# PacificBiosciences/minorseq

Hardware: AMD Instinct MI355X
Metric: aligned CCS reads/sec through juliet call+phase (higher is better)
Workload: dtype u3 symbols as bit planes / u32 counts / f64 p-values; 1 GPU; configs[2]: 100000 CCS reads x 3000 bp reference per GPU, pileup + Fisher-exact + phasing (96% major + four 1% minor haplotypes, sub 1.75e-4, del 1.3e-3, N 2e-2); every resident batch holds different reads; reads_per_gpu=100000, ref_columns_per_gpu=3000, parallelism=single GPU, batches_per_launch=8, launches_in_flight=4, resident_batches=32, variants_called=5, haplotypes=5, windows_verified_in_loop=270

## Files before the change

### minorseq_amd/csrc/kernels_pileup.hip

```cpp
#include <stdlib.h>
#include <string.h>

#include "call_eval.h"
#include "deviation_index.h"
#include "jl_internal.h"

namespace {


__device__ __forceinline__ uint32_t wave_sum(uint32_t v)
{
    v += (uint32_t)__builtin_amdgcn_update_dpp(0, (int)v, 0xB1, 0xF, 0xF, true);
    v += (uint32_t)__builtin_amdgcn_update_dpp(0, (int)v, 0x4E, 0xF, 0xF, true);
    v += (uint32_t)__builtin_amdgcn_update_dpp(0, (int)v, 0x141, 0xF, 0xF, true);
    v += (uint32_t)__builtin_amdgcn_update_dpp(0, (int)v, 0x140, 0xF, 0xF, true);
    v += (uint32_t)__builtin_amdgcn_update_dpp(0, (int)v, 0x142, 0xA, 0xF, false);
    v += (uint32_t)__builtin_amdgcn_update_dpp(0, (int)v, 0x143, 0xC, 0xF, false);
    return v;
}

typedef uint32_t u32x4 __attribute__((ext_vector_type(4)));

#define JL_CHUNK_META(ncols, startf, halo) ((uint32_t)(ncols) | ((uint32_t)(startf) << 4) | ((uint32_t)(halo) << 16))

typedef uint32_t u32x2 __attribute__((ext_vector_type(2)));
constexpr uint32_t plane_tile_bytes(int nq) { return 256u * 4u * (uint32_t)nq; }
constexpr uint32_t plane_flush_tiles(int nq) { return 1023u / (32u * (uint32_t)nq); }

template <int W, int NQ>
struct ptile_regs {
    uint32_t d[W + 2][3][NQ];
};

template <int W, int NQ, bool FAST>
__device__ __forceinline__ void load_ptile(ptile_regs<W, NQ> &r, const uint8_t JL_AS1 *planes, uint64_t plane_stride, uint32_t n_cols,
                                           uint32_t c0, uint32_t ncols, uint64_t off, bool need_halo)
{
#pragma unroll
    for (int j = 0; j < W + 2; ++j) {
        if (FAST && j >= 3) continue;
        const bool live = FAST ? true : (c0 + j < n_cols) && ((uint32_t)j < ncols || (need_halo && (uint32_t)j < ncols + 2u));
        if (live) {
            const uint8_t JL_AS1 *base = planes + (uint64_t)(c0 + j) * 3u * plane_stride + off;
#pragma unroll
            for (int k = 0; k < 3; ++k) {
                if (NQ == 2) {
                    const u32x2 v = __builtin_nontemporal_load((const u32x2 JL_AS1 *)(base + (uint64_t)k * plane_stride));
                    r.d[j][k][0] = v.x;
                    r.d[j][k][1] = v.y;
                } else {
                    const u32x4 v = __builtin_nontemporal_load((const u32x4 JL_AS1 *)(base + (uint64_t)k * plane_stride));
                    r.d[j][k][0] = v.x;
                    r.d[j][k][1] = v.y;
                    r.d[j][k][NQ - 2] = v.z;
                    r.d[j][k][NQ - 1] = v.w;
                }
            }
        } else {
#pragma unroll
            for (int q = 0; q < NQ; ++q) {
                r.d[j][0][q] = 0u;
                r.d[j][1][q] = r.d[j][2][q] = 0xFFFFFFFFu;
            }
        }
    }
}

template <int W, int NQ, bool FAST>
__device__ __forceinline__ void pileup_planes_stream(const uint8_t JL_AS1 *planes, uint64_t plane_stride, uint32_t n_cols,
                                                     uint32_t n_tiles, uint32_t c0, uint32_t ncols, uint32_t startf, bool need_halo,
                                                     const uint32_t (&g)[W + 2], uint32_t (*s_hist)[64], uint32_t (*s_col)[6],
                                                     uint32_t *s_match)
{
    constexpr uint32_t TILE = plane_tile_bytes(NQ);
    const uint32_t tid = threadIdx.x;
    const bool last_lane = (tid & 63u) == 63u;
    const uint64_t lane_off = (uint64_t)tid * 4u * NQ;
    uint32_t sh[W + 2], sl[W + 2];
#pragma unroll
    for (int j = 0; j < W + 2; ++j) {
        sh[j] = (g[j] & 2u) ? 0xFFFFFFFFu : 0u;
        sl[j] = (g[j] & 1u) ? 0xFFFFFFFFu : 0u;
    }

    uint32_t tile = blockIdx.y;
    ptile_regs<W, NQ> nxt;
    bool nxt_live = false;
    if (tile < n_tiles) {
        const uint64_t off = (uint64_t)tile * TILE + lane_off;
        nxt_live = off < plane_stride;
        if (nxt_live) load_ptile<W, NQ, FAST>(nxt, planes, plane_stride, n_cols, c0, ncols, off, need_halo);
    }

    while (tile < n_tiles) {
        uint32_t acc[W][6];
        uint32_t match[W];
#pragma unroll
        for (int j = 0; j < W; ++j) {
            match[j] = 0;
#pragma unroll
            for (int k = 0; k < 6; ++k) acc[j][k] = 0;
        }
        uint32_t reads = 0;

        for (uint32_t it = 0; it < plane_flush_tiles(NQ) && tile < n_tiles; ++it, tile += gridDim.y) {
            const ptile_regs<W, NQ> cur = nxt;
            const bool live = nxt_live;
            const uint32_t tn = tile + gridDim.y;
            nxt_live = false;
            if (tn < n_tiles) {
                const uint64_t off = (uint64_t)tn * TILE + lane_off;
                nxt_live = off < plane_stride;
                if (nxt_live) load_ptile<W, NQ, FAST>(nxt, planes, plane_stride, n_cols, c0, ncols, off, need_halo);
            }
            if (!live) continue;
            reads += 32u * NQ;
#pragma unroll
            for (int j = 0; j < W; ++j) {
                if (FAST ? j < 3 : (uint32_t)j < ncols) {
#pragma unroll
                    for (int q = 0; q < NQ; ++q) {
                        const uint32_t b0 = cur.d[j][0][q], b1 = cur.d[j][1][q], b2 = cur.d[j][2][q];
                        acc[j][0] += __popc(b0);
                        acc[j][1] += __popc(b1);
                        acc[j][2] += __popc(b2);
                        acc[j][3] += __popc(b0 & b1);
                        acc[j][4] += __popc(b0 & b2);
                        acc[j][5] += __popc(b1 & b2);
                    }
                }
            }
#pragma unroll
            for (int j = 0; j < W; ++j) {
                if (FAST ? j == 0 : (startf & (1u << j)) != 0) {
#pragma unroll
                    for (int q = 0; q < NQ; ++q) {
                        const uint32_t inv = cur.d[j][2][q] | cur.d[j + 1][2][q] | cur.d[j + 2][2][q];
                        const uint32_t x = (cur.d[j][1][q] ^ sh[j]) | (cur.d[j][0][q] ^ sl[j]) | (cur.d[j + 1][1][q] ^ sh[j + 1]) |
                                           (cur.d[j + 1][0][q] ^ sl[j + 1]) | (cur.d[j + 2][1][q] ^ sh[j + 2]) | (cur.d[j + 2][0][q] ^ sl[j + 2]);
                        match[j] += __popc(~(x | inv));
                        uint32_t rest = x & ~inv;
                        while (rest) {
                            const int b = __ffs((int)rest) - 1;
                            rest &= rest - 1;
                            const uint32_t idx = (((cur.d[j][1][q] >> b) & 1u) << 5) | (((cur.d[j][0][q] >> b) & 1u) << 4) |
                                                 (((cur.d[j + 1][1][q] >> b) & 1u) << 3) | (((cur.d[j + 1][0][q] >> b) & 1u) << 2) |
                                                 (((cur.d[j + 2][1][q] >> b) & 1u) << 1) | ((cur.d[j + 2][0][q] >> b) & 1u);
                            atomicAdd(&s_hist[j][idx], 1u);
                        }
                    }
                }
            }
        }

#pragma unroll
        for (int j = 0; j < W; ++j) {
            if (FAST && j >= 3) continue;
            const uint32_t nT = acc[j][3], nN = acc[j][4], nU = acc[j][5];
            const uint32_t nC = acc[j][0] - nT - nN, nG = acc[j][1] - nT - nU, nD = acc[j][2] - nN - nU;
            const uint32_t nA = reads - (nC + nG + nT + nD + nN + nU);
            const uint32_t p0 = wave_sum(nA | (nC << 16));
            const uint32_t p1 = wave_sum(nG | (nT << 16));
            const uint32_t p2 = wave_sum(nD | (nN << 16));
            const bool starts = FAST ? j == 0 : (startf & (1u << j)) != 0;
            uint32_t p3 = 0;
            if (starts) p3 = wave_sum(match[j]);
            if (last_lane && (uint32_t)j < ncols) {
                if (p0 & 0xFFFFu) atomicAdd(&s_col[j][0], p0 & 0xFFFFu);
                if (p0 >> 16) atomicAdd(&s_col[j][1], p0 >> 16);
                if (p1 & 0xFFFFu) atomicAdd(&s_col[j][2], p1 & 0xFFFFu);
                if (p1 >> 16) atomicAdd(&s_col[j][3], p1 >> 16);
                if (p2 & 0xFFFFu) atomicAdd(&s_col[j][4], p2 & 0xFFFFu);
                if (p2 >> 16) atomicAdd(&s_col[j][5], p2 >> 16);
                if (starts && p3) atomicAdd(&s_match[j], p3);
            }
        }
    }
}

template <int W, bool FOLD>
__device__ __forceinline__ void pileup_tail(uint32_t (*s_hist)[64], uint32_t (*s_col)[6], uint32_t *s_match, const uint32_t (&g)[W + 2],
                                            uint32_t c0, uint32_t ncols, uint32_t startf, uint32_t JL_AS1 *counts, uint32_t JL_AS1 *hist,
                                            const jl_win_fold *fold)
{
    const uint32_t tid = threadIdx.x;
    const bool excl = gridDim.y == 1;
    if (tid < W * 6) {
        const uint32_t j = tid / 6u, k = tid - j * 6u;
        const uint32_t v = s_col[j][k];
        if (j < ncols) {
            if (excl) counts[(uint64_t)(c0 + j) * 6u + k] = v;
            else if (v) atomicAdd((uint32_t *)(counts + (uint64_t)(c0 + j) * 6u + k), v);
        }
    }
    if (tid < W && (startf & (1u << tid))) {
        const uint32_t j = tid;
        const uint32_t seed = (g[j] << 4) | (g[j + 1] << 2) | g[j + 2];
        s_hist[j][seed] += s_match[j];
    }
    __syncthreads();
    for (uint32_t i = tid; i < W * 64; i += 256) {
        const uint32_t j = i >> 6;
        const uint32_t v = s_hist[j][i & 63u];
        if (startf & (1u << j)) {
            if (excl) hist[(uint64_t)(c0 + j) * 64u + (i & 63u)] = v;
            else if (v) atomicAdd((uint32_t *)(hist + (uint64_t)(c0 + j) * 64u + (i & 63u)), v);
        }
    }
    if (FOLD) {
        const jl_win_call &c = fold->c;
        if (blockIdx.x == 0 && tid == 0 && c.meta) {
            c.meta->n_occupied = 0;
            c.meta->overflow = 0;
            jl_phase_summary z = {0, 0, 0, 0, 0, 0, 0, 0};
            c.meta->summary = z;
        }
        const uint32_t wid = tid >> 6, lane = tid & 63u;
#pragma unroll
        for (int j = 0; j < W; ++j) {
            if (((uint32_t)j & 3u) != wid || !(startf & (1u << j))) continue;
            const uint32_t col = c0 + (uint32_t)j;
            const uint32_t h = s_hist[j][lane];
            for (uint32_t p = fold->col_head[col]; p != 0xFFFFFFFFu; p = fold->pos_next[p])
                jl_call_position<false>(c.A, p, col, h, c.pos_refcfg[p], c.pos_gene[p], c.pos_codon[p], c.drm, c.called, c.staged);
        }
    }
}

template <int W, int NQ, bool FOLD>
__device__ __forceinline__ void pileup_planes_body(const uint8_t JL_AS1 *planes, uint64_t plane_stride, uint32_t n_cols, uint32_t n_tiles,
                                                   const uint2 JL_AS1 *chunks, const uint32_t JL_AS1 *guess32, uint32_t JL_AS1 *counts,
                                                   uint32_t JL_AS1 *hist, const jl_win_fold *fold)
{
    __shared__ uint32_t s_hist[W][64];
    __shared__ uint32_t s_col[W][6];
    __shared__ uint32_t s_match[W];
    const uint32_t tid = threadIdx.x;
    const uint2 rec = chunks[blockIdx.x];
    const uint32_t c0 = rec.x;
    const uint32_t ncols = rec.y & 15u;
    const uint32_t startf = (rec.y >> 4) & 0xFFFu;
    const bool need_halo = ((rec.y >> 16) & 1u) != 0;
    constexpr int NG = (W + 2 + 3 + 3) / 4;
    uint32_t gw[NG];
#pragma unroll
    for (int k = 0; k < NG; ++k) gw[k] = guess32[(c0 >> 2) + k];
    uint32_t g[W + 2];
#pragma unroll
    for (int j = 0; j < W + 2; ++j) {
        const uint32_t b = (c0 & 3u) + (uint32_t)j;
        uint32_t word = gw[0];
#pragma unroll
        for (int k = 1; k < NG; ++k)
            if ((b >> 2) == (uint32_t)k) word = gw[k];
        g[j] = (word >> (8u * (b & 3u))) & 3u;
    }
    for (uint32_t i = tid; i < W * 64; i += 256) (&s_hist[0][0])[i] = 0;
    if (tid < W * 6) (&s_col[0][0])[tid] = 0;
    if (tid < W) s_match[tid] = 0;
    __syncthreads();
    if (W == 3 && rec.y == JL_CHUNK_META(3, 1, 0))
        pileup_planes_stream<W, NQ, true>(planes, plane_stride, n_cols, n_tiles, c0, ncols, startf, need_halo, g, s_hist, s_col, s_match);
    else
        pileup_planes_stream<W, NQ, false>(planes, plane_stride, n_cols, n_tiles, c0, ncols, startf, need_halo, g, s_hist, s_col, s_match);
    __syncthreads();
    pileup_tail<W, FOLD>(s_hist, s_col, s_match, g, c0, ncols, startf, counts, hist, fold);
}

template <int W, int NQ>
__global__ __launch_bounds__(256) void pileup_planes_kernel(const uint8_t *__restrict__ planes, uint64_t plane_stride, uint32_t n_cols,
                                                            uint32_t n_tiles, const uint2 *__restrict__ chunks,
                                                            const uint32_t *__restrict__ guess32, uint32_t *__restrict__ counts,
                                                            uint32_t *__restrict__ hist)
{
    pileup_planes_body<W, NQ, false>((const uint8_t JL_AS1 *)planes, plane_stride, n_cols, n_tiles, (const uint2 JL_AS1 *)chunks,
                                     (const uint32_t JL_AS1 *)guess32, (uint32_t JL_AS1 *)counts, (uint32_t JL_AS1 *)hist, nullptr);
}

template <int W, int NQ>
__global__ __launch_bounds__(256) void pileup_planes_group_kernel(jl_pileup_group_args args)
{
    const jl_win_pileup &w = args.w[blockIdx.z];
    if (blockIdx.x >= w.n_chunks) return;
    pileup_planes_body<W, NQ, false>((const uint8_t JL_AS1 *)w.msa, w.plane_stride, w.n_cols, w.n_tiles, (const uint2 JL_AS1 *)w.chunks,
                                     (const uint32_t JL_AS1 *)w.guess32, (uint32_t JL_AS1 *)w.counts, (uint32_t JL_AS1 *)w.hist, nullptr);
}

template <int W, int NQ>
__global__ __launch_bounds__(256) void pileup_fold_kernel(jl_win_pileup w, jl_win_fold f)
{
    pileup_planes_body<W, NQ, true>((const uint8_t JL_AS1 *)w.msa, w.plane_stride, w.n_cols, w.n_tiles, (const uint2 JL_AS1 *)w.chunks,
                                    (const uint32_t JL_AS1 *)w.guess32, (uint32_t JL_AS1 *)w.counts, (uint32_t JL_AS1 *)w.hist, &f);
}

template <int W, int NQ>
__global__ __launch_bounds__(256) void pileup_fold_group_kernel(jl_pileup_fold_group_args args)
{
    const jl_win_pileup &w = args.w[blockIdx.z];
    if (blockIdx.x >= w.n_chunks) return;
    pileup_planes_body<W, NQ, true>((const uint8_t JL_AS1 *)w.msa, w.plane_stride, w.n_cols, w.n_tiles, (const uint2 JL_AS1 *)w.chunks,
                                    (const uint32_t JL_AS1 *)w.guess32, (uint32_t JL_AS1 *)w.counts, (uint32_t JL_AS1 *)w.hist, &args.f[blockIdx.z]);
}

#ifndef JL_IX_FOLD_DEPTH
#define JL_IX_FOLD_DEPTH 8
#endif
template <int DEPTH>
__device__ __forceinline__ void index_stream(const uint32_t JL_AS1 *list, uint32_t E, uint32_t (*s_hist)[64], uint32_t (*s_col)[6])
{
    static_assert(DEPTH >= 1 && DEPTH <= 8, "rounds held in registers");
    constexpr uint32_t FLUSH_BATCHES = JL_IX_FLUSH_ROUNDS / (uint32_t)DEPTH;
    static_assert(FLUSH_BATCHES >= 1u && FLUSH_BATCHES * (uint32_t)DEPTH <= JL_IX_FLUSH_ROUNDS, "a 9-bit field never above 511");
    const uint32_t tid = threadIdx.x;
    const bool last_lane = (tid & 63u) == 63u;
    const u32x4 JL_AS1 *src = (const u32x4 JL_AS1 *)list;
    const uint32_t n_rounds = (E + 4u * 256u - 1u) / (4u * 256u);
    u32x4 buf[DEPTH];
#pragma unroll
    for (int k = 0; k < DEPTH; ++k) {
        buf[k] = u32x4{0u, 0u, 0u, 0u};
        if (((uint32_t)k * 256u + tid) * 4u < E) buf[k] = __builtin_nontemporal_load(src + (size_t)k * 256u + tid);
    }
    uint32_t r = 0;
    while (r < n_rounds) {
        unsigned long long acc[3] = {0ull, 0ull, 0ull};
        for (uint32_t it = 0; it < FLUSH_BATCHES && r < n_rounds; ++it, r += (uint32_t)DEPTH) {
#pragma unroll
            for (int k = 0; k < DEPTH; ++k) {
                if (r + (uint32_t)k >= n_rounds) break;
                const u32x4 cur = buf[k];
                const uint32_t first = ((r + (uint32_t)k) * 256u + tid) * 4u;
                const uint32_t nfirst = first + (uint32_t)DEPTH * 4u * 256u;
                if (nfirst < E) buf[k] = __builtin_nontemporal_load(src + (size_t)(r + (uint32_t)k + (uint32_t)DEPTH) * 256u + tid);
                const uint32_t e4[4] = {cur.x, cur.y, cur.z, cur.w};
#pragma unroll
                for (int i = 0; i < 4; ++i) {
                    if (first + (uint32_t)i >= E) continue;
                    const uint32_t e = e4[i];
                    const uint32_t a = (e >> 6) & 7u, b = (e >> 3) & 7u, c = e & 7u;
                    acc[0] += 1ull << (JL_IX_FIELD_BITS * a);
                    acc[1] += 1ull << (JL_IX_FIELD_BITS * b);
                    acc[2] += 1ull << (JL_IX_FIELD_BITS * c);
                    if ((e & 0x124u) == 0u) atomicAdd(&s_hist[0][(a << 4) | (b << 2) | c], 1u);
                }
            }
        }
#pragma unroll
        for (int j = 0; j < 3; ++j) {
            const uint32_t m = (1u << JL_IX_FIELD_BITS) - 1u;
            uint32_t p[3];
#pragma unroll
            for (int k = 0; k < 3; ++k)
                p[k] = wave_sum(((uint32_t)(acc[j] >> (JL_IX_FIELD_BITS * 2u * k)) & m) | (((uint32_t)(acc[j] >> (JL_IX_FIELD_BITS * (2u * k + 1u))) & m) << 16));
            if (last_lane) {
#pragma unroll
                for (int k = 0; k < 3; ++k) {
                    if (p[k] & 0xFFFFu) atomicAdd(&s_col[j][2 * k], p[k] & 0xFFFFu);
                    if (p[k] >> 16) atomicAdd(&s_col[j][2 * k + 1], p[k] >> 16);
                }
            }
        }
    }
}

__device__ __forceinline__ void index_dense_stream(const uint8_t JL_AS1 *planes, uint64_t plane_stride, uint32_t c0, const uint32_t (&g)[5],
                                                   uint32_t (*s_hist)[64], uint32_t (*s_col)[6], uint32_t *s_match)
{
    const uint32_t tid = threadIdx.x;
    const bool last_lane = (tid & 63u) == 63u;
    const uint32_t n_words = (uint32_t)(plane_stride / 4u);
    const uint32_t JL_AS1 *base = (const uint32_t JL_AS1 *)(planes + (uint64_t)c0 * 3u * plane_stride);
    const uint64_t row = plane_stride / 4u;
    uint32_t acc[3][6], match = 0, reads = 0;
#pragma unroll
    for (int j = 0; j < 3; ++j)
#pragma unroll
        for (int k = 0; k < 6; ++k) acc[j][k] = 0;
    for (uint32_t w = tid; w < n_words; w += 256u) {
        uint32_t d[3][3];
#pragma unroll
        for (int j = 0; j < 3; ++j)
#pragma unroll
            for (int k = 0; k < 3; ++k) d[j][k] = base[(uint64_t)(3 * j + k) * row + w];
        reads += 32u;
        uint32_t inv = 0, x = 0;
#pragma unroll
        for (int j = 0; j < 3; ++j) {
            const uint32_t b0 = d[j][0], b1 = d[j][1], b2 = d[j][2];
            acc[j][0] += __popc(b0);
            acc[j][1] += __popc(b1);
            acc[j][2] += __popc(b2);
            acc[j][3] += __popc(b0 & b1);
            acc[j][4] += __popc(b0 & b2);
            acc[j][5] += __popc(b1 & b2);
            inv |= b2;
            x |= (b1 ^ ((g[j] & 2u) ? 0xFFFFFFFFu : 0u)) | (b0 ^ ((g[j] & 1u) ? 0xFFFFFFFFu : 0u));
        }
        match += __popc(~(x | inv));
        uint32_t rest = x & ~inv;
        while (rest) {
            const int b = __ffs((int)rest) - 1;
            rest &= rest - 1;
            const uint32_t idx = (((d[0][1] >> b) & 1u) << 5) | (((d[0][0] >> b) & 1u) << 4) | (((d[1][1] >> b) & 1u) << 3) |
                                 (((d[1][0] >> b) & 1u) << 2) | (((d[2][1] >> b) & 1u) << 1) | ((d[2][0] >> b) & 1u);
            atomicAdd(&s_hist[0][idx], 1u);
        }
    }
#pragma unroll
    for (int j = 0; j < 3; ++j) {
        const uint32_t nT = acc[j][3], nN = acc[j][4], nU = acc[j][5];
        const uint32_t nC = acc[j][0] - nT - nN, nG = acc[j][1] - nT - nU, nD = acc[j][2] - nN - nU;
        const uint32_t nA = reads - (nC + nG + nT + nD + nN + nU);
        const uint32_t v[6] = {wave_sum(nA), wave_sum(nC), wave_sum(nG), wave_sum(nT), wave_sum(nD), wave_sum(nN)};
        if (last_lane) {
#pragma unroll
            for (int k = 0; k < 6; ++k)
                if (v[k]) atomicAdd(&s_col[j][k], v[k]);
        }
    }
    const uint32_t ms = wave_sum(match);
    if (last_lane && ms) atomicAdd(&s_match[0], ms);
}

template <bool FOLD>
__device__ __forceinline__ void pileup_index_body(const uint8_t JL_AS1 *planes, uint64_t plane_stride, uint32_t n_reads, const uint4 JL_AS1 *tab,
                                                  const uint32_t JL_AS1 *entries, const uint8_t JL_AS1 *seed, uint32_t JL_AS1 *counts,
                                                  uint32_t JL_AS1 *hist, const jl_win_fold *fold)
{
    __shared__ uint32_t s_hist[3][64];
    __shared__ uint32_t s_col[3][6];
    __shared__ uint32_t s_match[3];
    const uint32_t tid = threadIdx.x;
    const uint4 rec = tab[blockIdx.x];
    const uint32_t c0 = rec.x;
    const uint32_t g[5] = {seed[c0] & 3u, seed[c0 + 1u] & 3u, seed[c0 + 2u] & 3u, 0u, 0u};
    for (uint32_t i = tid; i < 3 * 64; i += 256) (&s_hist[0][0])[i] = 0;
    if (tid < 3 * 6) (&s_col[0][0])[tid] = 0;
    if (tid < 3) s_match[tid] = 0;
    __syncthreads();
    if (rec.z != 0xFFFFFFFFu) {
        index_stream<FOLD ? JL_IX_FOLD_DEPTH : 1>(entries + rec.y, rec.z, s_hist, s_col);
        if (tid < 3) atomicAdd(&s_col[tid][g[tid]], n_reads - rec.z);
        if (tid == 3) s_match[0] = n_reads - rec.z;
    } else {
        index_dense_stream(planes, plane_stride, c0, g, s_hist, s_col, s_match);
    }
    __syncthreads();
    pileup_tail<3, FOLD>(s_hist, s_col, s_match, g, c0, 3u, 1u, counts, hist, fold);
}

#define JL_INDEX_BODY(FOLD, w, f)                                                                                                     \
    pileup_index_body<FOLD>((const uint8_t JL_AS1 *)(w).msa, (w).plane_stride, (w).n_reads, (const uint4 JL_AS1 *)(w).tab,            \
                            (const uint32_t JL_AS1 *)(w).entries, (const uint8_t JL_AS1 *)(w).seed, (uint32_t JL_AS1 *)(w).counts,     \
                            (uint32_t JL_AS1 *)(w).hist, f)

__global__ __launch_bounds__(256) void pileup_index_kernel(jl_win_index w) { JL_INDEX_BODY(false, w, nullptr); }
__global__ __launch_bounds__(256) void pileup_index_fold_kernel(jl_win_index w, jl_win_fold f) { JL_INDEX_BODY(true, w, &f); }
__global__ __launch_bounds__(256) void pileup_index_group_kernel(jl_index_group_args args)
{
    const jl_win_index &w = args.w[blockIdx.z];
    if (blockIdx.x >= w.n_plain) return;
    JL_INDEX_BODY(false, w, nullptr);
}
__global__ __launch_bounds__(256) void pileup_index_fold_group_kernel(jl_index_fold_group_args args)
{
    const jl_win_index &w = args.w[blockIdx.z];
    if (blockIdx.x >= w.n_plain) return;
    JL_INDEX_BODY(true, w, &args.f[blockIdx.z]);
}
#undef JL_INDEX_BODY

__global__ __launch_bounds__(64) void guess_kernel(const uint8_t *__restrict__ planes, uint64_t plane_stride,
                                                   uint32_t n_cols, uint8_t *__restrict__ guess)
{
    const uint32_t c = blockIdx.x;
    if (c >= n_cols) return;
    const uint32_t lane = threadIdx.x;
    uint32_t nA = 0, nC = 0, nG = 0, nT = 0;
    const uint64_t off = (uint64_t)lane * 4u;
    if (off < plane_stride) {
        const uint8_t *base = planes + (uint64_t)c * 3u * plane_stride + off;
        const uint32_t b0 = *reinterpret_cast<const uint32_t *>(base);
        const uint32_t b1 = *reinterpret_cast<const uint32_t *>(base + plane_stride);
        const uint32_t b2 = *reinterpret_cast<const uint32_t *>(base + 2u * plane_stride);
        nA = __popc(~b2 & ~b1 & ~b0);
        nC = __popc(~b2 & ~b1 & b0);
        nG = __popc(~b2 & b1 & ~b0);
        nT = __popc(~b2 & b1 & b0);
    }
    const uint32_t p0 = wave_sum(nA | (nC << 16));
    const uint32_t p1 = wave_sum(nG | (nT << 16));
    if (lane == 63) {
        uint32_t best = 0, bv = p0 & 0xFFFFu;
        if ((p0 >> 16) > bv) { bv = p0 >> 16; best = 1; }
        if ((p1 & 0xFFFFu) > bv) { bv = p1 & 0xFFFFu; best = 2; }
        if ((p1 >> 16) > bv) { bv = p1 >> 16; best = 3; }
        guess[c] = (uint8_t)best;
    }
}

}

const char *jl_pileup_kernel_name(void) { return "pileup_planes_kernel"; }

static int planes_nq(const jl_ctx *ctx, bool grouped) { return ctx->pileup_w == 3 && (grouped || ctx->plane_stride >= 32768u) ? 4 : 2; }
static uint32_t planes_tiles(const jl_ctx *ctx, bool grouped)
{
    const uint32_t tile = plane_tile_bytes(planes_nq(ctx, grouped));
    return (uint32_t)((ctx->plane_stride + tile - 1) / tile);
}
static int planes_slot(const jl_ctx *ctx) { return ctx->pileup_w == 3 ? (planes_nq(ctx, false) == 4 ? 0 : 1) : 2; }

void jl_launch_guess(jl_ctx *ctx, hipStream_t st)
{
    hipLaunchKernelGGL(guess_kernel, dim3(ctx->n_cols), dim3(64), 0, st, ctx->d_msa, ctx->plane_stride, ctx->n_cols, ctx->d_guess);
}

void jl_prepare_pileup(jl_ctx *ctx)
{
    const int idx = planes_slot(ctx);
    if (ctx->pileup_blocks_per_cu[idx] > 0) return;
    const void *fn = idx == 0 ? (const void *)pileup_planes_kernel<3, 4> : idx == 1 ? (const void *)pileup_planes_kernel<3, 2>
                                                                                    : (const void *)pileup_planes_kernel<6, 2>;
    int per_cu = 0;
    if (hipOccupancyMaxActiveBlocksPerMultiprocessor(&per_cu, fn, 256, 0) != hipSuccess || per_cu < 1) per_cu = 2;
    if (per_cu > 8) per_cu = 8;
    ctx->pileup_blocks_per_cu[idx] = per_cu;
}

uint32_t jl_pileup_rsplit(jl_ctx *ctx)
{
    jl_prepare_pileup(ctx);
    const uint32_t n_chunks = ctx->n_chunks ? ctx->n_chunks : 1u;
    const uint32_t n_tiles = planes_tiles(ctx, false);
    const int per_cu = ctx->pileup_blocks_per_cu[planes_slot(ctx)];
    const uint32_t target = 256u * (uint32_t)per_cu * (n_tiles >= 64 ? 4u : 1u);
    uint32_t rsplit = target / n_chunks;
    if (rsplit > n_tiles) rsplit = n_tiles;
    if (rsplit < 1) rsplit = 1;
    if (rsplit > 65535u) rsplit = 65535u;
    return rsplit;
}

bool jl_pileup_needs_zero(jl_ctx *ctx) { return jl_pileup_rsplit(ctx) != 1u; }

void jl_launch_pileup(jl_ctx *ctx, hipStream_t st)
{
    const uint32_t rsplit = jl_pileup_rsplit(ctx);
    const uint32_t nt = planes_tiles(ctx, false);
#define JL_LAUNCH_PLANES(W, NQ)                                                                                                       \
    hipLaunchKernelGGL((pileup_planes_kernel<W, NQ>), dim3(ctx->n_chunks, rsplit), dim3(256), 0, st, ctx->d_msa, ctx->plane_stride,   \
                       ctx->n_cols, nt, ctx->d_chunks.as<const uint2>(), ctx->d_guess.as<const uint32_t>(), ctx->d_counts, ctx->d_hist)
    if (ctx->pileup_w == 6) JL_LAUNCH_PLANES(6, 2);
    else if (planes_nq(ctx, false) == 4) JL_LAUNCH_PLANES(3, 4);
    else JL_LAUNCH_PLANES(3, 2);
#undef JL_LAUNCH_PLANES
}

bool jl_fold_enabled(void) { return !jl_env().no_fold_call; }
bool jl_pileup_can_fold(jl_ctx *ctx) { return jl_fold_enabled() && ctx->P != 0 && jl_pileup_rsplit(ctx) == 1u; }

void jl_fill_win_fold(jl_ctx *ctx, const jl_win_call *call, jl_win_fold *f)
{
    f->c = *call;
    f->col_head = ctx->d_col_head;
    f->pos_next = ctx->d_pos_next;
}

void jl_launch_pileup_fold(jl_ctx *ctx, hipStream_t st, const jl_win_call *call)
{
    jl_win_pileup w;
    jl_win_fold f;
    w.msa = ctx->d_msa;
    w.plane_stride = ctx->plane_stride;
    w.n_cols = ctx->n_cols;
    w.n_tiles = planes_tiles(ctx, false);
    w.n_chunks = ctx->n_chunks;
    w.pad_ = 0;
    w.chunks = ctx->d_chunks.as<const uint2>();
    w.guess32 = ctx->d_guess.as<const uint32_t>();
    w.counts = ctx->d_counts;
    w.hist = ctx->d_hist;
    jl_fill_win_fold(ctx, call, &f);
    if (ctx->pileup_w == 6) hipLaunchKernelGGL((pileup_fold_kernel<6, 2>), dim3(ctx->n_chunks, 1), dim3(256), 0, st, w, f);
    else if (planes_nq(ctx, false) == 4) hipLaunchKernelGGL((pileup_fold_kernel<3, 4>), dim3(ctx->n_chunks, 1), dim3(256), 0, st, w, f);
    else hipLaunchKernelGGL((pileup_fold_kernel<3, 2>), dim3(ctx->n_chunks, 1), dim3(256), 0, st, w, f);
}

int jl_launch_pileup_fold_group(jl_ctx *const *ctxs, uint32_t n_win, const jl_win_pileup *h_wins, const jl_win_fold *h_fold, uint32_t max_chunks, hipStream_t st)
{
    if (n_win == 0 || n_win > JL_GROUP_MAX) return JL_ERR_ARG;
    for (uint32_t k = 1; k < n_win; ++k)
        if (ctxs[k]->pileup_w != ctxs[0]->pileup_w) return JL_ERR_ARG;
    jl_pileup_fold_group_args args;
    memset(&args, 0, sizeof args);
    memcpy(args.w, h_wins, sizeof(jl_win_pileup) * n_win);
    memcpy(args.f, h_fold, sizeof(jl_win_fold) * n_win);
    if (ctxs[0]->pileup_w == 3) hipLaunchKernelGGL((pileup_fold_group_kernel<3, 4>), dim3(max_chunks, 1, n_win), dim3(256), 0, st, args);
    else hipLaunchKernelGGL((pileup_fold_group_kernel<6, 2>), dim3(max_chunks, 1, n_win), dim3(256), 0, st, args);
    return JL_OK;
}

void jl_fill_win_pileup(jl_ctx *ctx, jl_win_pileup *w)
{
    w->msa = ctx->d_msa;
    w->plane_stride = ctx->plane_stride;
    w->n_cols = ctx->n_cols;
    w->n_tiles = planes_tiles(ctx, true);
    w->n_chunks = ctx->n_chunks;
    w->pad_ = 0;
    w->chunks = ctx->d_chunks.as<const uint2>();
    w->guess32 = ctx->d_guess.as<const uint32_t>();
    w->counts = ctx->d_counts;
    w->hist = ctx->d_hist;
}

int jl_launch_pileup_group(jl_ctx *const *ctxs, uint32_t n_win, const jl_win_pileup *h_wins, uint32_t max_chunks, hipStream_t st)
{
    if (n_win == 0 || n_win > JL_GROUP_WINDOWS_MAX) return JL_ERR_ARG;
    for (uint32_t k = 1; k < n_win; ++k)
        if (ctxs[k]->pileup_w != ctxs[0]->pileup_w) return JL_ERR_ARG;
    jl_pileup_group_args args;
    memset(&args, 0, sizeof args);
    memcpy(args.w, h_wins, sizeof(jl_win_pileup) * n_win);
    if (ctxs[0]->pileup_w == 3) hipLaunchKernelGGL((pileup_planes_group_kernel<3, 4>), dim3(max_chunks, 1, n_win), dim3(256), 0, st, args);
    else hipLaunchKernelGGL((pileup_planes_group_kernel<6, 2>), dim3(max_chunks, 1, n_win), dim3(256), 0, st, args);
    return JL_OK;
}

void jl_fill_win_index(jl_ctx *ctx, jl_win_index *w)
{
    w->msa = ctx->d_msa;
    w->plane_stride = ctx->plane_stride;
    w->n_reads = (uint32_t)ctx->n_reads;
    w->n_plain = ctx->ix_n_plain;
    w->tab = ctx->d_ix_tab;
    w->entries = ctx->d_ix_entries;
    w->seed = ctx->d_ix_seed;
    w->counts = ctx->d_counts;
    w->hist = ctx->d_hist;
}

void jl_fill_win_pileup_rest(jl_ctx *ctx, bool grouped, jl_win_pileup *w)
{
    jl_fill_win_pileup(ctx, w);
    w->n_tiles = planes_tiles(ctx, grouped);
    w->n_chunks = ctx->ix_n_rest;
    w->chunks = ctx->d_ix_rest.as<const uint2>();
}

void jl_launch_pileup_index(jl_ctx *ctx, hipStream_t st, const jl_win_call *call)
{
    jl_win_index wi;
    jl_win_pileup w;
    jl_win_fold f;
    jl_fill_win_index(ctx, &wi);
    jl_fill_win_pileup_rest(ctx, false, &w);
    if (call) jl_fill_win_fold(ctx, call, &f);
    if (call) hipLaunchKernelGGL(pileup_index_fold_kernel, dim3(wi.n_plain), dim3(256), 0, st, wi, f);
    else hipLaunchKernelGGL(pileup_index_kernel, dim3(wi.n_plain), dim3(256), 0, st, wi);
    if (!w.n_chunks) return;
    const int nq = planes_nq(ctx, false);
    if (call) {
        if (nq == 4) hipLaunchKernelGGL((pileup_fold_kernel<3, 4>), dim3(w.n_chunks, 1), dim3(256), 0, st, w, f);
        else hipLaunchKernelGGL((pileup_fold_kernel<3, 2>), dim3(w.n_chunks, 1), dim3(256), 0, st, w, f);
    } else {
        const uint32_t rsplit = jl_pileup_rsplit(ctx);
        if (nq == 4) hipLaunchKernelGGL((pileup_planes_kernel<3, 4>), dim3(w.n_chunks, rsplit), dim3(256), 0, st, w.msa, w.plane_stride, w.n_cols, w.n_tiles, w.chunks, w.guess32, w.counts, w.hist);
        else hipLaunchKernelGGL((pileup_planes_kernel<3, 2>), dim3(w.n_chunks, rsplit), dim3(256), 0, st, w.msa, w.plane_stride, w.n_cols, w.n_tiles, w.chunks, w.guess32, w.counts, w.hist);
    }
}

int jl_launch_pileup_index_group(jl_ctx *const *ctxs, uint32_t n_win, const jl_win_index *h_wins, const jl_win_fold *h_fold, uint32_t max_plain, hipStream_t st)
{
    (void)ctxs;
    if (n_win == 0 || n_win > JL_GROUP_MAX || max_plain == 0) return JL_ERR_ARG;
    if (h_fold) {
        jl_index_fold_group_args args;
        memset(&args, 0, sizeof args);
        memcpy(args.w, h_wins, sizeof(jl_win_index) * n_win);
        memcpy(args.f, h_fold, sizeof(jl_win_fold) * n_win);
        hipLaunchKernelGGL(pileup_index_fold_group_kernel, dim3(max_plain, 1, n_win), dim3(256), 0, st, args);
    } else {
        jl_index_group_args args;
        memset(&args, 0, sizeof args);
        memcpy(args.w, h_wins, sizeof(jl_win_index) * n_win);
        hipLaunchKernelGGL(pileup_index_group_kernel, dim3(max_plain, 1, n_win), dim3(256), 0, st, args);
    }
    return JL_OK;
}

#ifdef JL_TUNING
extern "C" __attribute__((visibility("default"))) int jl_tuning_pileup_shape(jl_ctx *ctx, uint32_t *out)
{
    if (!ctx || !out || !ctx->plan_valid) return JL_ERR_ARG;
    std::vector<uint2> recs(ctx->n_chunks);
    if (hipSetDevice(ctx->device) != hipSuccess || hipStreamSynchronize(ctx->stream) != hipSuccess ||
        (ctx->n_chunks && hipMemcpy(recs.data(), ctx->d_chunks.as<const uint2>(), recs.size() * sizeof(uint2), hipMemcpyDeviceToHost) != hipSuccess))
        return JL_ERR_DEVICE;
    uint32_t n_fast = 0, n_halo = 0;
    for (const uint2 &r : recs) {
        n_fast += ctx->pileup_w == 3 && r.y == JL_CHUNK_META(3, 1, 0);
        n_halo += (r.y >> 16) & 1u;
    }
    const uint32_t v[12] = {ctx->pileup_w, (uint32_t)planes_nq(ctx, false), planes_tiles(ctx, false), (uint32_t)planes_nq(ctx, true),
                            planes_tiles(ctx, true), ctx->n_chunks, jl_pileup_rsplit(ctx), (uint32_t)jl_pileup_can_fold(ctx),
                            (uint32_t)ctx->pileup_blocks_per_cu[planes_slot(ctx)], n_fast, n_halo, plane_flush_tiles(planes_nq(ctx, false))};
    memcpy(out, v, sizeof v);
    return JL_OK;
}
#endif
```

Baseline: 9.179 billion reads/s.

## Issue index-stream loads and fold metadata fetch before shared-memory setup

The index pileup body now issues its first DEPTH vector loads of the entry list, and loads the first fold position's head, refcfg, gene and codon, before zeroing shared memory and syncing, so these global latencies overlap the block prologue. The non-fold path's stream depth rises from 1 to a configurable 4. Loads use clamped addresses instead of branches, with a separate no-refill batch for the last rounds. The cost is more registers held across the sync, which may lower occupancy, plus some redundant clamped loads.

```diff
diff --git a/minorseq_amd/csrc/kernels_pileup.hip b/minorseq_amd/csrc/kernels_pileup.hip
--- a/minorseq_amd/csrc/kernels_pileup.hip
+++ b/minorseq_amd/csrc/kernels_pileup.hip
@@ -178,10 +178,11 @@
     }
 }
 
+struct jl_fold_first { uint32_t p, refcfg, gene, codon; };
 template <int W, bool FOLD>
 __device__ __forceinline__ void pileup_tail(uint32_t (*s_hist)[64], uint32_t (*s_col)[6], uint32_t *s_match, const uint32_t (&g)[W + 2],
                                             uint32_t c0, uint32_t ncols, uint32_t startf, uint32_t JL_AS1 *counts, uint32_t JL_AS1 *hist,
-                                            const jl_win_fold *fold)
+                                            const jl_win_fold *fold, const jl_fold_first *first = nullptr)
 {
     const uint32_t tid = threadIdx.x;
     const bool excl = gridDim.y == 1;
@@ -221,8 +222,10 @@
             if (((uint32_t)j & 3u) != wid || !(startf & (1u << j))) continue;
             const uint32_t col = c0 + (uint32_t)j;
             const uint32_t h = s_hist[j][lane];
-            for (uint32_t p = fold->col_head[col]; p != 0xFFFFFFFFu; p = fold->pos_next[p])
-                jl_call_position<false>(c.A, p, col, h, c.pos_refcfg[p], c.pos_gene[p], c.pos_codon[p], c.drm, c.called, c.staged);
+            bool hoisted = first != nullptr && j == 0;
+            for (uint32_t p = hoisted ? first->p : fold->col_head[col]; p != 0xFFFFFFFFu; p = fold->pos_next[p], hoisted = false)
+                jl_call_position<false>(c.A, p, col, h, hoisted ? first->refcfg : (uint32_t)c.pos_refcfg[p], hoisted ? first->gene : c.pos_gene[p],
+                                        hoisted ? first->codon : c.pos_codon[p], c.drm, c.called, c.staged);
         }
     }
 }
@@ -305,8 +308,56 @@
 #ifndef JL_IX_FOLD_DEPTH
 #define JL_IX_FOLD_DEPTH 8
 #endif
+#ifndef JL_IX_PLAIN_DEPTH
+#define JL_IX_PLAIN_DEPTH 4
+#endif
 template <int DEPTH>
-__device__ __forceinline__ void index_stream(const uint32_t JL_AS1 *list, uint32_t E, uint32_t (*s_hist)[64], uint32_t (*s_col)[6])
+__device__ __forceinline__ void index_stream_issue(u32x4 (&buf)[DEPTH], const uint32_t JL_AS1 *list, uint32_t E)
+{
+    static_assert(DEPTH >= 1 && DEPTH <= 8, "rounds held in registers");
+    const uint32_t tid = threadIdx.x;
+    const u32x4 JL_AS1 *src = (const u32x4 JL_AS1 *)list;
+#pragma unroll
+    for (int k = 0; k < DEPTH; ++k) buf[k] = u32x4{0u, 0u, 0u, 0u};
+    if (E == 0u) return;
+#pragma unroll
+    for (int k = 0; k < DEPTH; ++k) {
+        const uint32_t slot = (uint32_t)k * 256u + tid;
+        buf[k] = __builtin_nontemporal_load(src + (slot * 4u < E ? slot : 0u));
+    }
+}
+
+template <int DEPTH, bool REFILL>
+__device__ __forceinline__ void index_batch(u32x4 (&buf)[DEPTH], const u32x4 JL_AS1 *src, uint32_t E, uint32_t r, uint32_t n_rounds,
+                                            unsigned long long (&acc)[3], uint32_t (*s_hist)[64])
+{
+    const uint32_t tid = threadIdx.x;
+#pragma unroll
+    for (int k = 0; k < DEPTH; ++k) {
+        if (r + (uint32_t)k >= n_rounds) break;
+        const u32x4 cur = buf[k];
+        const uint32_t first = ((r + (uint32_t)k) * 256u + tid) * 4u;
+        if (REFILL) {
+            const uint32_t nslot = (r + (uint32_t)k + (uint32_t)DEPTH) * 256u + tid;
+            buf[k] = __builtin_nontemporal_load(src + (nslot * 4u < E ? nslot : 0u));
+        }
+        const uint32_t e4[4] = {cur.x, cur.y, cur.z, cur.w};
+#pragma unroll
+        for (int i = 0; i < 4; ++i) {
+            if (first + (uint32_t)i >= E) continue;
+            const uint32_t e = e4[i];
+            const uint32_t a = (e >> 6) & 7u, b = (e >> 3) & 7u, c = e & 7u;
+            acc[0] += 1ull << (JL_IX_FIELD_BITS * a);
+            acc[1] += 1ull << (JL_IX_FIELD_BITS * b);
+            acc[2] += 1ull << (JL_IX_FIELD_BITS * c);
+            if ((e & 0x124u) == 0u) atomicAdd(&s_hist[0][(a << 4) | (b << 2) | c], 1u);
+        }
+    }
+}
+
+template <int DEPTH>
+__device__ __forceinline__ void index_stream(u32x4 (&buf)[DEPTH], const uint32_t JL_AS1 *list, uint32_t E, uint32_t (*s_hist)[64],
+                                             uint32_t (*s_col)[6])
 {
     static_assert(DEPTH >= 1 && DEPTH <= 8, "rounds held in registers");
     constexpr uint32_t FLUSH_BATCHES = JL_IX_FLUSH_ROUNDS / (uint32_t)DEPTH;
@@ -315,35 +366,12 @@
     const bool last_lane = (tid & 63u) == 63u;
     const u32x4 JL_AS1 *src = (const u32x4 JL_AS1 *)list;
     const uint32_t n_rounds = (E + 4u * 256u - 1u) / (4u * 256u);
-    u32x4 buf[DEPTH];
-#pragma unroll
-    for (int k = 0; k < DEPTH; ++k) {
-        buf[k] = u32x4{0u, 0u, 0u, 0u};
-        if (((uint32_t)k * 256u + tid) * 4u < E) buf[k] = __builtin_nontemporal_load(src + (size_t)k * 256u + tid);
-    }
     uint32_t r = 0;
     while (r < n_rounds) {
         unsigned long long acc[3] = {0ull, 0ull, 0ull};
         for (uint32_t it = 0; it < FLUSH_BATCHES && r < n_rounds; ++it, r += (uint32_t)DEPTH) {
-#pragma unroll
-            for (int k = 0; k < DEPTH; ++k) {
-                if (r + (uint32_t)k >= n_rounds) break;
-                const u32x4 cur = buf[k];
-                const uint32_t first = ((r + (uint32_t)k) * 256u + tid) * 4u;
-                const uint32_t nfirst = first + (uint32_t)DEPTH * 4u * 256u;
-                if (nfirst < E) buf[k] = __builtin_nontemporal_load(src + (size_t)(r + (uint32_t)k + (uint32_t)DEPTH) * 256u + tid);
-                const uint32_t e4[4] = {cur.x, cur.y, cur.z, cur.w};
-#pragma unroll
-                for (int i = 0; i < 4; ++i) {
-                    if (first + (uint32_t)i >= E) continue;
-                    const uint32_t e = e4[i];
-                    const uint32_t a = (e >> 6) & 7u, b = (e >> 3) & 7u, c = e & 7u;
-                    acc[0] += 1ull << (JL_IX_FIELD_BITS * a);
-                    acc[1] += 1ull << (JL_IX_FIELD_BITS * b);
-                    acc[2] += 1ull << (JL_IX_FIELD_BITS * c);
-                    if ((e & 0x124u) == 0u) atomicAdd(&s_hist[0][(a << 4) | (b << 2) | c], 1u);
-                }
-            }
+            if (r + (uint32_t)DEPTH < n_rounds) index_batch<DEPTH, true>(buf, src, E, r, n_rounds, acc, s_hist);
+            else index_batch<DEPTH, false>(buf, src, E, r, n_rounds, acc, s_hist);
         }
 #pragma unroll
         for (int j = 0; j < 3; ++j) {
@@ -430,23 +458,35 @@
     __shared__ uint32_t s_hist[3][64];
     __shared__ uint32_t s_col[3][6];
     __shared__ uint32_t s_match[3];
+    constexpr int DEPTH = FOLD ? JL_IX_FOLD_DEPTH : JL_IX_PLAIN_DEPTH;
     const uint32_t tid = threadIdx.x;
     const uint4 rec = tab[blockIdx.x];
     const uint32_t c0 = rec.x;
+    const bool indexed = rec.z != 0xFFFFFFFFu;
+    jl_fold_first first = {0xFFFFFFFFu, 0u, 0u, 0u};
+    const bool evaluates = FOLD && (tid >> 6) == 0u;
+    if (evaluates) first.p = fold->col_head[c0];
+    u32x4 buf[DEPTH];
+    index_stream_issue<DEPTH>(buf, entries + rec.y, indexed ? rec.z : 0u);
     const uint32_t g[5] = {seed[c0] & 3u, seed[c0 + 1u] & 3u, seed[c0 + 2u] & 3u, 0u, 0u};
+    if (evaluates && first.p != 0xFFFFFFFFu) {
+        first.refcfg = fold->c.pos_refcfg[first.p];
+        first.gene = fold->c.pos_gene[first.p];
+        first.codon = fold->c.pos_codon[first.p];
+    }
     for (uint32_t i = tid; i < 3 * 64; i += 256) (&s_hist[0][0])[i] = 0;
     if (tid < 3 * 6) (&s_col[0][0])[tid] = 0;
     if (tid < 3) s_match[tid] = 0;
     __syncthreads();
-    if (rec.z != 0xFFFFFFFFu) {
-        index_stream<FOLD ? JL_IX_FOLD_DEPTH : 1>(entries + rec.y, rec.z, s_hist, s_col);
+    if (indexed) {
+        index_stream<DEPTH>(buf, entries + rec.y, rec.z, s_hist, s_col);
         if (tid < 3) atomicAdd(&s_col[tid][g[tid]], n_reads - rec.z);
         if (tid == 3) s_match[0] = n_reads - rec.z;
     } else {
         index_dense_stream(planes, plane_stride, c0, g, s_hist, s_col, s_match);
     }
     __syncthreads();
-    pileup_tail<3, FOLD>(s_hist, s_col, s_match, g, c0, 3u, 1u, counts, hist, fold);
+    pileup_tail<3, FOLD>(s_hist, s_col, s_match, g, c0, 3u, 1u, counts, hist, fold, FOLD ? &first : nullptr);
 }
 
 #define JL_INDEX_BODY(FOLD, w, f)                                                                                                     \
```

Result: faster. 9.307 billion reads/s (median of 6 runs) (+1.4%).
